# junyanz/interactive-deep-colorization

Hardware: NVIDIA H100
Metric: net_forward images/sec @256x256 (higher is better)
Workload: dtype f16x2-split operands, f32 accumulate (ab within 1e-3 of the f32 reference)

## Files before the change

include/idc_b200.h:

```cpp
#ifndef IDC_B200_H_
#define IDC_B200_H_

#include <stddef.h>
#include <stdint.h>

#ifdef __cplusplus
extern "C" {
#endif

typedef struct idc_ctx idc_ctx;

enum {
  IDC_OK = 0,
  IDC_ERR_ARG = -1,
  IDC_ERR_CUDA = -2,
  IDC_ERR_STATE = -3,
  IDC_ERR_KEY = -4,
  IDC_ERR_UNSUPPORTED = -5,
  IDC_ERR_WATCHDOG = -6,
  IDC_ERR_RANGE = -7
};

enum {
  IDC_FLAG_DIST = 1u << 0,
// ... 71 lines not shown
                         int mask_f32, int l_mode, const double* L, int h, int w, uint8_t* rgb, void* stream);

int idc_resize_u8_linear(int device, int h_src, int w_src, const uint8_t* src, int h_dst, int w_dst, uint8_t* dst,
                         void* stream);
int idc_cubic_lab2rgb_u8(int device, int h_in, int w_in, const double* ab, int h, int w, const double* L, uint8_t* rgb,
                         void* stream);
int idc_gamut_ab(int device, double L, int gamut_size, int D, uint8_t* rgb, uint8_t* mask, void* stream);

typedef struct { int64_t off; int32_t h, w; } idc_photo;
#define IDC_MAX_PHOTOS 128
#define IDC_MAX_PHOTO_SIDE 16777216
#define IDC_MAX_PHOTO_X 16384
int idc_photo_prep(int device, int n, const idc_photo* photos, const uint8_t* src, int X, float* L_mc, uint8_t* rgb,
                   void* stream);
int idc_photo_render(int device, int n, const idc_photo* photos, const uint8_t* src, int X, const double* lab,
                     uint8_t* out, void* stream);
int idc_hint_raster(int device, int n, int h, int w, int count, const void* block, float* ab, float* mask, void* stream);
int idc_rgb_sse(int device, int n, int h, int w, const uint8_t* a, const uint8_t* b, int64_t* sse, void* stream);

int idc_act_exponent(idc_ctx* ctx, const char* name, int* exp_out);
int idc_num_acts(idc_ctx* ctx);
const char* idc_act_name(idc_ctx* ctx, int i);
int idc_act_absmax(idc_ctx* ctx, const char* name, int n, float* out_host);
int idc_set_act_range(idc_ctx* ctx, const char* name, double max_abs);
int idc_get_activation(idc_ctx* ctx, const char* name, float* out_nchw, size_t out_floats,
                       int* c, int* h, int* w);
int idc_set_activation(idc_ctx* ctx, const char* name, int n, const float* in_nchw);
int idc_run_op(idc_ctx* ctx, const char* op_name, int n, void* stream);
int idc_num_ops(idc_ctx* ctx);
const char* idc_op_name(idc_ctx* ctx, int i);
int idc_set_profiling(idc_ctx* ctx, int enable);
int idc_get_profile(idc_ctx* ctx, float* ms, int max_slots);
double idc_op_flops(idc_ctx* ctx, int i);
int idc_last_launch_count(idc_ctx* ctx);
int idc_graph_captures(idc_ctx* ctx);
double idc_flops_per_image(idc_ctx* ctx);

const char* idc_last_error(idc_ctx* ctx);
int idc_destroy(idc_ctx* ctx);

#ifdef __cplusplus
}
#endif
#endif
```

interactive_deep_colorization_b200/_lib.py:

```python
import ctypes
import os

import numpy as np

_HERE = os.path.dirname(os.path.abspath(__file__))
LIB_PATH = os.path.join(_HERE, "lib", "libidc_b200.so")
if os.environ.get("IDC_B200_LIB"):
    LIB_PATH = os.environ["IDC_B200_LIB"]

IDC_OK = 0
ERR_ARG, ERR_CUDA, ERR_STATE, ERR_KEY, ERR_UNSUPPORTED, ERR_WATCHDOG, ERR_RANGE = -1, -2, -3, -4, -5, -6, -7
FLAG_DIST = 1 << 0
FLAG_ENGINE_SIMT = 1 << 1
FLAG_FAST_FP16 = 1 << 2
FLAG_GLOBAL_HINTS = 1 << 3
FLAG_NO_GRAPH = 1 << 4
FLAG_KEEP_CONV10 = 1 << 5
FLAG_CAFFE313 = 1 << 6
F32, F64, I64 = 0, 1, 2
MAX_HINTS = 1024
MAX_PHOTOS = 128
MAX_PHOTO_SIDE = 1 << 24
MAX_PHOTO_X = 16384
HINT_HDR_BYTES = 16
# ... 28 lines not shown
    ("idc_ab_reccs", _c.c_int, [_P, _c.c_int, _c.c_int, _c.c_int, _c.c_int, _c.c_int, _c.c_int, _P, _P, _P, _P]),
    ("idc_ab_reccs_pmf", _c.c_int, [_c.c_int, _P, _c.c_int, _c.c_int, _c.c_int, _P, _P, _P, _P]),
    ("idc_caffe313_pred_ab", _c.c_int, [_P, _c.c_int, _c.c_float, _P, _P]),
    ("idc_caffe313_dist_pixel", _c.c_int, [_P, _c.c_int, _c.c_int, _c.c_int, _c.c_float, _P]),
    ("idc_caffe313_dist_map", _c.c_int, [_P, _c.c_int, _c.c_float, _P, _P]),
    ("idc_negentropy", _c.c_int, [_c.c_int, _c.c_int, _c.c_int, _c.c_int, _P, _P, _P]),
    ("idc_dist_negentropy", _c.c_int, [_P, _c.c_int, _P]),
    ("idc_lab2rgb_u8", _c.c_int, [_c.c_int, _c.c_int, _c.c_int, _c.c_int, _P, _P, _P, _P]),
    ("idc_rgb2lab_f64", _c.c_int, [_c.c_int, _c.c_int, _c.c_int, _c.c_int, _P, _P, _P]),
    ("idc_global_stats", _c.c_int, [_c.c_int, _c.c_int, _c.c_int, _P, _P, _P, _P]),
    ("idc_zoom_lab2rgb_u8", _c.c_int, [_c.c_int, _c.c_int, _c.c_int, _P, _c.c_int, _c.c_int, _P, _P, _P]),
    ("idc_render_planes_u8", _c.c_int, [_c.c_int, _c.c_int, _c.c_int, _P, _c.c_int, _c.c_int, _P, _c.c_int, _c.c_int,
                                        _P, _c.c_int, _c.c_int, _P, _P]),
    ("idc_resize_u8_linear", _c.c_int, [_c.c_int, _c.c_int, _c.c_int, _P, _c.c_int, _c.c_int, _P, _P]),
    ("idc_cubic_lab2rgb_u8", _c.c_int, [_c.c_int, _c.c_int, _c.c_int, _P, _c.c_int, _c.c_int, _P, _P, _P]),
    ("idc_photo_prep", _c.c_int, [_c.c_int, _c.c_int, _P, _P, _c.c_int, _P, _P, _P]),
    ("idc_photo_render", _c.c_int, [_c.c_int, _c.c_int, _P, _P, _c.c_int, _P, _P, _P]),
    ("idc_hint_raster", _c.c_int, [_c.c_int, _c.c_int, _c.c_int, _c.c_int, _c.c_int, _P, _P, _P, _P]),
    ("idc_rgb_sse", _c.c_int, [_c.c_int, _c.c_int, _c.c_int, _c.c_int, _P, _P, _P, _P]),
    ("idc_get_activation", _c.c_int, [_P, _c.c_char_p, _P, _c.c_size_t, _c.POINTER(_c.c_int),
                                      _c.POINTER(_c.c_int), _c.POINTER(_c.c_int)]),
    ("idc_set_activation", _c.c_int, [_P, _c.c_char_p, _c.c_int, _P]),
    ("idc_act_exponent", _c.c_int, [_P, _c.c_char_p, _c.POINTER(_c.c_int)]),
    ("idc_num_acts", _c.c_int, [_P]),
    ("idc_act_name", _c.c_char_p, [_P, _c.c_int]),
    ("idc_act_absmax", _c.c_int, [_P, _c.c_char_p, _c.c_int, _c.POINTER(_c.c_float)]),
    ("idc_set_act_range", _c.c_int, [_P, _c.c_char_p, _c.c_double]),
    ("idc_run_op", _c.c_int, [_P, _c.c_char_p, _c.c_int, _P]),
    ("idc_num_ops", _c.c_int, [_P]),
    ("idc_op_name", _c.c_char_p, [_P, _c.c_int]),
    ("idc_set_profiling", _c.c_int, [_P, _c.c_int]),
    ("idc_get_profile", _c.c_int, [_P, _c.POINTER(_c.c_float), _c.c_int]),
    ("idc_op_flops", _c.c_double, [_P, _c.c_int]),
    ("idc_last_launch_count", _c.c_int, [_P]),
    ("idc_flops_per_image", _c.c_double, [_P]),
    ("idc_last_error", _c.c_char_p, [_P]),
    ("idc_destroy", _c.c_int, [_P]),
]

_lib = None


class IdcError(RuntimeError):
    def __init__(self, code, msg):
        RuntimeError.__init__(self, "idc_b200 error %d: %s" % (code, msg))
        self.code = code


def load():
    global _lib
    if _lib is not None:
        return _lib
    if not os.path.isfile(LIB_PATH):
        raise ImportError("libidc_b200.so not built (%s missing); run `python -c 'import __graft_entry__ as g; g.build()'` "
                          "or `make -C interactive_deep_colorization_b200/csrc`" % LIB_PATH)
    lib = ctypes.CDLL(LIB_PATH)
    for name, res, args in SYMBOLS:
        fn = getattr(lib, name)
        fn.restype = res
        fn.argtypes = args
    _lib = lib
    return lib


def check(ctx, rc):
    if rc != IDC_OK:
# ... 3 lines not shown
```

interactive_deep_colorization_b200/csrc/idc_api.cu:

```cuda
#include <math.h>
#include <stdarg.h>
#include <stdio.h>
#include <string.h>

#include <algorithm>
#include <cmath>

#include "idc_internal.h"

using namespace idc;

struct idc_ctx : public idc::Ctx {};

namespace {

int fail(Ctx* c, int code, const char* fmt, ...) {
  char buf[512];
  va_list ap;
  va_start(ap, fmt);
  vsnprintf(buf, sizeof(buf), fmt, ap);
  va_end(ap);
  if (c) c->err = buf;
  return code;
}
// ... 1572 lines not shown
  return IDC_OK;
}

int idc_get_profile(idc_ctx* c, float* ms, int max_slots) {
  if (!c || !ms) return IDC_ERR_ARG;
  const int slots = (int)c->ops.size() + 2;
  if (max_slots < slots) return fail(c, IDC_ERR_ARG, "need %d slots", slots);
  CUDA_TRY(c, cudaSetDevice(c->dev));
  CUDA_TRY(c, cudaDeviceSynchronize());
  const int rc = take_device_flags(c, "device pipeline watchdog fired (code %d)");
  if (rc != IDC_OK) return rc;
  for (int i = 0; i < slots; ++i) ms[i] = 0.f;
  int runs = 0;
  for (auto& ev : c->prof_runs) {
    if ((int)ev.size() == slots + 1) {
      for (int i = 0; i < slots; ++i) {
        float t = 0.f;
        cudaEventElapsedTime(&t, ev[i].get(), ev[i + 1].get());
        ms[i] += t;
      }
      runs++;
    }
    for (Event& e : ev) c->prof_pool.push_back(std::move(e));
  }
  c->prof_runs.clear();
  if (runs) for (int i = 0; i < slots; ++i) ms[i] /= runs;
  return slots;
}

double idc_op_flops(idc_ctx* c, int i) {
  return (c && i >= 0 && i < (int)c->ops.size()) ? c->ops[i].flops_per_image : 0.0;
}

extern "C" int idc_debug_graph_timing(idc_ctx* c, int enable, float* ms) {
  if (!c) return IDC_ERR_ARG;
  CUDA_TRY(c, cudaSetDevice(c->dev));
  if (enable && !c->dbg_ev[0].get()) {
    Event ev[2];
    CUDA_TRY(c, cudaEventCreate(ev[0].put()));
    CUDA_TRY(c, cudaEventCreate(ev[1].put()));
    c->dbg_ev[0] = std::move(ev[0]);
    c->dbg_ev[1] = std::move(ev[1]);
  }
  c->dbg_graph_timing = enable != 0 && c->dbg_ev[0].get();
  if (ms) *ms = c->dbg_graph_ms;
  return IDC_OK;
}

int idc_num_ops(idc_ctx* c) { return c ? (int)c->ops.size() : 0; }
const char* idc_op_name(idc_ctx* c, int i) {
  return (c && i >= 0 && i < (int)c->ops.size()) ? c->ops[i].name.c_str() : nullptr;
}
int idc_last_launch_count(idc_ctx* c) { return c ? c->launch_count : 0; }
int idc_graph_captures(idc_ctx* c) { return c ? c->graph_captures : 0; }

double idc_flops_per_image(idc_ctx* c) {
  if (!c) return 0;
  double f = 2.0 * c->H * c->W * 64.0 * 36.0 + 2.0 * c->H * c->W * 2.0 * 128.0;
  for (auto& op : c->ops) f += op.flops_per_image;
  return f;
}

const char* idc_last_error(idc_ctx* c) { return c ? c->err.c_str() : "null ctx"; }

int idc_destroy(idc_ctx* c) {
  if (!c) return IDC_ERR_ARG;
// ... 8 lines not shown
```

interactive_deep_colorization_b200/csrc/idc_internal.h:

```cpp
#pragma once
#include <cuda.h>
#include <cuda_fp16.h>
#include <cuda_runtime.h>
#include <stdint.h>

#include <map>
#include <memory>
#include <string>
#include <utility>
#include <vector>

#include "../../include/idc_b200.h"

namespace idc {

template <typename H, auto Release>
class Owner {
 public:
  Owner() = default;
  Owner(Owner&& o) noexcept { std::swap(h_, o.h_); }
  Owner& operator=(Owner&& o) noexcept { std::swap(h_, o.h_); return *this; }
  ~Owner() { reset(); }
  H get() const { return h_; }
  H* put() { reset(); return &h_; }
// ... 169 lines not shown
  Stream own_stream;
  std::unique_ptr<HostPipeStreams> pipe;
  std::unique_ptr<SideBranch> side;
  int image_n = 0;
  std::unique_ptr<HintBlock> hints;
  int graph_captures = 0;
  GraphExec graph_exec;
  const void* graph_ptrs[8] = {nullptr};
  float graph_maskcent = 0.f;
  int launch_count = 0;
  int graph_launches = 0;
  bool chain = false;
  bool gadd_active = false;
  int last_n = 0;
  DevMem<double> d_reccs;
  DevMem<float> d_negent;
  DevMem<float> d_dist313;
  bool dist_resident = false;
  int dist_valid_n = 0;
  bool click_mode = false;
  std::unique_ptr<ClickBlock> click;
  bool click_served = false;
  bool profiling = false;
  std::vector<std::vector<Event>> prof_runs;
  std::vector<Event> prof_pool;
  std::string err;
};

cudaError_t simt_run_op(Ctx* c, ConvOp& op, int n, cudaStream_t st);
int umma_plan_op(Ctx* c, ConvOp& op);
cudaError_t umma_run_op(Ctx* c, ConvOp& op, int n, float* out_ab_fused, float out_mult, cudaStream_t st, int img0 = 0,
                        int max_ctas = 0);
bool umma_op_uses_split_k(const ConvOp& op);

cudaError_t launch_conv1_1(Ctx* c, int n, const float* L, const float* ab, const float* mask,
                           float maskcent, cudaStream_t st, int img0 = 0);
cudaError_t launch_conv1_1_umma(Ctx* c, int n, const float* L, const float* ab, const float* mask, float maskcent,
                                cudaStream_t st, int img0 = 0);
cudaError_t conv1_1_umma_pack(Ctx* c);
constexpr size_t kHintHdrBytes = 16;
constexpr size_t kHintBlockBytes = kHintHdrBytes + (size_t)IDC_MAX_HINTS * sizeof(idc_hint);
cudaError_t launch_hint_raster(Ctx* c, int n, int H, int W, const char* hints_dev, float* ab, float* mask,
                               cudaStream_t st);
cudaError_t launch_gamut(double L, int gamut_size, int D, int A, uint8_t* rgb, uint8_t* mask, cudaStream_t st);
cudaError_t launch_out_head(Ctx* c, int n, float* out_ab, cudaStream_t st);
cudaError_t launch_softmax529(Ctx* c, int n, float* out_dist, cudaStream_t st);
cudaError_t launch_lab2rgb(Ctx* c, int n, int h, int w, const float* L, float l_offset, const float* ab,
                           uint8_t* rgb, cudaStream_t st, double* abq = nullptr);
cudaError_t launch_decode313(Ctx* c, int n, float T, float* out_ab, cudaStream_t st);
cudaError_t launch_dist313_pixel(Ctx* c, int img, int y, int x, float S, float* out313_dev, cudaStream_t st);
cudaError_t launch_dist313_map(Ctx* c, int n, float S, float* out_dev, cudaStream_t st);
cudaError_t launch_negentropy(int n, int bins, int hw, const float* dist, float* out, cudaStream_t st);
cudaError_t launch_ab_reccs(const float* pmf, size_t bin_stride, const float* pts_dev, int K, int max_iter,
                            int n_init, double* out_dev, cudaStream_t st, const int* dyn = nullptr);
cudaError_t launch_click_pmf(Ctx* c, const int* click_dev, int n_img, int* out_hdr, float* out_pmf, cudaStream_t st);
cudaError_t launch_global_stats(int h, int w, const uint8_t* rgb, const float* pts, float* out316, cudaStream_t st);
cudaError_t launch_rgb2lab(int n, int h, int w, const uint8_t* rgb, double* lab, cudaStream_t st);
cudaError_t launch_render_planes(const double* ab, int ab_order, int ab_f32, const double* mask, int mask_f32, int l_mode,
                                 const double* L, int hin, int win, int H, int W, uint8_t* rgb, cudaStream_t st);
cudaError_t launch_resize_linear_u8(const uint8_t* src, int hs, int ws, uint8_t* dst, int hd, int wd, cudaStream_t st);
cudaError_t launch_cubic_lab2rgb(const double* ab, int hin, int win, const double* L, int H, int W, uint8_t* rgb,
                                 cudaStream_t st);
cudaError_t launch_photo_prep(int n, const idc_photo* table, const uint8_t* src, int X, float* L_mc, uint8_t* rgb,
                              cudaStream_t st);
cudaError_t launch_photo_render(int n, const idc_photo* table, const uint8_t* src, int X, const double* lab, uint8_t* out,
                                cudaStream_t st);
// ... 155 lines not shown
```

interactive_deep_colorization_b200/csrc/idc_umma.cu:

```cuda
#include <stdio.h>
#include <stdlib.h>

#include "idc_internal.h"

namespace idc {

constexpr int kBM = 128;
constexpr int kBK = 64;
constexpr int kThreads = 384;
constexpr int kProdRegs = 40;
constexpr int kMathRegs = 232;
constexpr int kMathThreads = 256;

struct UmmaParams {
  const CUtensorMap* amaps;
  const int4* kblk;
  int nkb, ncls;
  int chunk_kb;
  int split_k;
  float* ws;
  int* counters;
  int n_img, tiles_y, tiles_x, n_tiles_n, total_tiles;
  int hbox, wbox, wshift;
  int Hl, Wl, cout_pad;
// ... 184 lines not shown
}
__device__ __forceinline__ bool f16_top(uint32_t m) {
  return ((m & 0xFFFFu) >= kF16MaxBits) | ((m >> 16) >= kF16MaxBits);
}

__device__ __forceinline__ void split_h(float v, __half& hi, __half& lo) {
  v = fminf(fmaxf(v, -65504.f), 65504.f);
  hi = __float2half_rn(v);
  lo = __float2half_rn(v - __half2float(hi));
}

__device__ __forceinline__ int frag_col(int i, int lane) { return 8 * (i >> 2) + 2 * (lane & 3) + (i & 1); }

constexpr int kHaloW = 10, kHaloH = 18;
constexpr int kHaloPlane = (kHaloW * kHaloH * 128 + 1023) / 1024 * 1024;


template <int BN, int MT, int CG, bool SPLIT, bool HALO>
struct SmemPlan {
  static constexpr int kABytes = MT * kBM * kBK * 2;
  static constexpr int kAStage = HALO ? 0 : kABytes;
  static constexpr int kBBytes = BN * kBK * 2;
  static constexpr int kStageBytes = (SPLIT ? 2 : 1) * (kAStage + kBBytes);
  static constexpr int kHaloSlot = (SPLIT ? 2 : 1) * kHaloPlane;
  static constexpr int kHaloBytes = HALO ? 2 * kHaloSlot : 0;
  static constexpr int kOutRow = 64 * 2 + 16;
  static constexpr int kOutWarp = 16 * kOutRow;
  static constexpr int kOutStage = 8 * kOutWarp;
  static constexpr int kTail = 3 * BN * 4 + 272 * 4 + 256;
  static constexpr int kBudget = 232448 - 1024 - kTail - kOutStage - kHaloBytes;
  static constexpr int kStages = kBudget / kStageBytes >= 4 ? 4 : kBudget / kStageBytes;
  static constexpr int kTotal = kStages * kStageBytes + kHaloBytes + kOutStage + kTail + 1024;
  static_assert(kStages >= 2, "need at least a double-buffered operand ring");
  static_assert(MT * BN <= 128, "register budget: chunk + tile accumulators of MT*BN columns per math thread pair");
  static_assert(!HALO || MT == 1, "halo tiles are single 16x8-pixel M-tiles");
  static_assert(CG == 1 || CG == 2, "clusters of one or two CTAs");
};

template <int BN, int MT, int CG, bool SPLIT, bool HALO>
__global__ void __launch_bounds__(kThreads, 1)
umma_conv_kernel(const __grid_constant__ CUtensorMap bmap_hi, const __grid_constant__ CUtensorMap bmap_lo,
                 const __grid_constant__ UmmaParams p) {
  using SP = SmemPlan<BN, MT, CG, SPLIT, HALO>;
  constexpr int STAGES = SP::kStages;
  constexpr int R = BN / 2;
  constexpr bool PAIR = CG == 2;
  extern __shared__ uint8_t smem_raw[];
  uint8_t* smem = reinterpret_cast<uint8_t*>((reinterpret_cast<uintptr_t>(smem_raw) + 1023) & ~uintptr_t(1023));
  uint8_t* s_halo = smem + STAGES * SP::kStageBytes;
  uint8_t* s_out = s_halo + SP::kHaloBytes;
  float* s_bias = reinterpret_cast<float*>(s_out + SP::kOutStage);
  float* s_scale = s_bias + BN;
  float* s_shift = s_scale + BN;
  float* s_head = s_shift + BN;
  uint64_t* full_bar = reinterpret_cast<uint64_t*>(s_head + 272);
  uint64_t* empty_bar = full_bar + 4;
  uint64_t* afull_bar = full_bar + 8;
  uint64_t* aempty_bar = full_bar + 10;

  const int warp = threadIdx.x >> 5, lane = threadIdx.x & 31;
  const uint32_t cta_rank = PAIR ? cluster_ctarank() : 0u;

  if (p.wout) {
    for (int i = threadIdx.x; i < 256; i += kThreads) s_head[i] = p.wout[i];
    if (threadIdx.x < 2) s_head[256 + threadIdx.x] = p.bout[threadIdx.x];
  }
  if (threadIdx.x == 32) {
    prefetch_tmap(&bmap_hi);
    if (SPLIT) prefetch_tmap(&bmap_lo);
    for (int i = 0; i < p.n_amaps; ++i) prefetch_tmap(p.amaps + i);
  }
  if (threadIdx.x == 0) {
    for (int s = 0; s < STAGES; ++s) {
      mbar_init(smem_u32(&full_bar[s]), 1);
      mbar_init(smem_u32(&empty_bar[s]), 8 * CG);
    }
    if (HALO)
      for (int a = 0; a < 2; ++a) {
        mbar_init(smem_u32(&afull_bar[a]), 1);
        mbar_init(smem_u32(&aempty_bar[a]), 8);
      }
    asm volatile("fence.mbarrier_init.release.cluster;" ::: "memory");
  }
  if (PAIR) cluster_sync_all(); else __syncthreads();
  pdl_launch_dependents();
  pdl_wait();

  const int tiles_per_img = p.tiles_y * p.tiles_x;
  const int S = p.split_k;
  const int n_items = p.total_tiles * S;
  const int w0 = blockIdx.x / CG, wstep = gridDim.x / CG;

  if (warp < 4) {
    asm volatile("setmaxnreg.dec.sync.aligned.u32 %0;" ::"n"(kProdRegs));
    if (warp == 0) {
      int stage = 0;
      uint32_t phase = 0;
      uint32_t hcount = 0;
      for (int w = w0; w < n_items; w += wstep) {
        const int tile = w / S, ks = w - tile * S;
        const int kbeg = (ks * p.nkb) / S, kend = ((ks + 1) * p.nkb) / S;
        int r = tile;
        const int nt = r % p.n_tiles_n;
        r /= p.n_tiles_n;
        const int cls = r % p.ncls;
        r /= p.ncls;
        if (PAIR) r = 2 * r + (int)cta_rank;
        const int img_rel = r / tiles_per_img;
        r -= img_rel * tiles_per_img;
        const int img = p.img0 + img_rel;
        const int y0 = (r / p.tiles_x) * (p.hbox * MT), x0 = (r % p.tiles_x) * p.wbox;
        const int brow = cls * p.cout_pad + nt * BN + (int)cta_rank * (BN / CG);
        const int4* kb = p.kblk + cls * p.nkb;
        for (int k = kbeg; k < kend; ++k) {
          if (HALO && k % 9 == 0) {
            const uint32_t slot = hcount & 1, hphase = (hcount >> 1) & 1;
            ++hcount;
            mbar_wait(smem_u32(&aempty_bar[slot]), hphase ^ 1, p.err, 6);
            if (elect_one()) {
              const uint32_t fa = smem_u32(&afull_bar[slot]);
              const uint32_t sh = smem_u32(s_halo + slot * SP::kHaloSlot);
              const int c0 = (k / 9) * kBK;
// ... 18 lines not shown
            }
            if (PAIR) {
              tma_load_2d_mc(sb, &bmap_hi, fb, kcol, brow);
              if (SPLIT) tma_load_2d_mc(sb + SP::kBBytes, &bmap_lo, fb, kcol, brow);
            } else {
              tma_load_2d(sb, &bmap_hi, fb, kcol, brow);
              if (SPLIT) tma_load_2d(sb + SP::kBBytes, &bmap_lo, fb, kcol, brow);
            }
          }
          __syncwarp();
          if (++stage == STAGES) { stage = 0; phase ^= 1; }
        }
      }
    }
  } else {
    asm volatile("setmaxnreg.inc.sync.aligned.u32 %0;" ::"n"(kMathRegs));
    const int et = threadIdx.x - 128;
    const int wg = et >> 7;
    const int wi = (et >> 5) & 3;
    const uint32_t wbuf = smem_u32(s_out) + (uint32_t)(et >> 5) * SP::kOutWarp;
    auto release = [&](uint64_t* bar) {
      __syncwarp();
      if (lane == 0) {
        mbar_arrive(smem_u32(bar));
        if (PAIR) mbar_arrive_remote(smem_u32(bar), cta_rank ^ 1u);
      }
    };
    int stage = 0;
    uint32_t phase = 0;
    uint32_t hcount = 0;
    int staged_key = -1;
    bool sat = false;
    for (int w = w0; w < n_items; w += wstep) {
      const int tile = w / S, ks = w - tile * S;
      const int kbeg = (ks * p.nkb) / S, kend = ((ks + 1) * p.nkb) / S;
      int r = tile;
      const int nt = r % p.n_tiles_n;
      r /= p.n_tiles_n;
      const int cls = r % p.ncls;
      r /= p.ncls;
      if (PAIR) r = 2 * r + (int)cta_rank;
      const int img_rel = r / tiles_per_img;
      r -= img_rel * tiles_per_img;
      const int img = p.img0 + img_rel;
      const int ty0 = (r / p.tiles_x) * (p.hbox * MT), tx0 = (r % p.tiles_x) * p.wbox;
      const int n0 = nt * BN;
      const int vkey = p.gadd ? (img * p.n_tiles_n + nt) : nt;
      if (vkey != staged_key) {
        asm volatile("bar.sync 1, 256;" ::: "memory");
        for (int i = et; i < BN; i += kMathThreads) {
          s_bias[i] = p.bias[n0 + i];
          s_scale[i] = p.scale[n0 + i];
          const int gi = img < p.n_img ? img : p.n_img - 1;
          s_shift[i] = p.shift[n0 + i] + (p.gadd ? p.gadd[(size_t)gi * p.gadd_ld + n0 + i] * p.gadd_mult : 0.f);
        }
        asm volatile("bar.sync 1, 256;" ::: "memory");
        staged_key = vkey;
      }

      float acc[MT][R];
#pragma unroll
      for (int m = 0; m < MT; ++m)
#pragma unroll
        for (int j = 0; j < R; ++j) acc[m][j] = 0.f;
      for (int k0 = kbeg; k0 < kend; k0 += p.chunk_kb) {
        const int k1 = (k0 + p.chunk_kb < kend) ? k0 + p.chunk_kb : kend;
        float part[MT][R];
#pragma unroll
        for (int m = 0; m < MT; ++m)
#pragma unroll
          for (int j = 0; j < R; ++j) part[m][j] = 0.f;
        int prev = -1;
        for (int k = k0; k < k1; ++k) {
          uint32_t hslot = 0;
          if (HALO) {
            if (k % 9 == 0) {
              mbar_wait(smem_u32(&afull_bar[hcount & 1]), (hcount >> 1) & 1, p.err, 7);
              ++hcount;
            }
            hslot = (hcount - 1) & 1;
          }
          mbar_wait(smem_u32(&full_bar[stage]), phase, p.err, 3);
          const uint32_t st0 = smem_u32(smem + stage * SP::kStageBytes);
          const uint32_t sb = st0 + (SPLIT ? 2 : 1) * SP::kAStage;
          const uint64_t b_hi = make_sw128_desc(sb), b_lo = make_sw128_desc(sb + SP::kBBytes);
          uint32_t ha = 0;
          if (HALO) {
            const int4 e = __ldg(p.kblk + k);
            ha = smem_u32(s_halo + hslot * SP::kHaloSlot) + (uint32_t)((e.z + wg * 8) * kHaloW + e.w) * 128u;
          }
          wgmma_fence();
#pragma unroll
          for (int m = 0; m < MT; ++m) {
            const uint32_t sa = st0 + (uint32_t)(wg * MT + m) * (64 * 128);
            const uint64_t a_hi = HALO ? make_sw128_desc(ha, kHaloW * 128) : make_sw128_desc(sa);
            const uint64_t a_lo = HALO ? make_sw128_desc(ha + kHaloPlane, kHaloW * 128) : make_sw128_desc(sa + SP::kABytes);
            uint32_t first = (k == k0) ? 0u : 1u;
// ... 58 lines not shown
          if (q == ks) continue;
          const float* rp = p.ws + (size_t)(tile * S + q) * R * kMathThreads + et;
#pragma unroll
          for (int i = 0; i < R; ++i)
            if ((i >> 4) % S == ks) acc[0][i] += __ldcg(rp + (size_t)i * kMathThreads);
        }
      }

      const float neg_slope = p.act == ACT_RELU ? 0.f : (p.act == ACT_LEAKY02 ? 0.2f : 1.f);
      unsigned own = ~0u;
      if (S > 1) {
        own = 0u;
#pragma unroll
        for (int pc = 0; pc < BN / 32; ++pc) own |= (pc % S == ks ? 1u : 0u) << pc;
      }
#pragma unroll
      for (int m = 0; m < MT; ++m) {
        const int blk = (wg * MT + m) * 64;
#pragma unroll
        for (int i = 0; i < R; ++i) {
          const int c = frag_col(i, lane);
          const float t = acc[m][i] + s_bias[c];
          acc[m][i] = fmaf(fmaxf(t, neg_slope * t), s_scale[c], s_shift[c]);
        }
        int ry[2], rx[2];
        bool ok[2];
#pragma unroll
        for (int h = 0; h < 2; ++h) {
          const int rr = blk + wi * 16 + (lane >> 2) + 8 * h;
          ry[h] = ty0 + (rr >> p.wshift);
          rx[h] = tx0 + (rr & (p.wbox - 1));
          ok[h] = ry[h] < p.Hl && rx[h] < p.Wl && img < p.n_img;
        }
        if (p.wout) {
          float h0[2] = {0.f, 0.f}, h1[2] = {0.f, 0.f};
#pragma unroll
          for (int i = 0; i < R; ++i) {
            const int c = frag_col(i, lane), h = (i >> 1) & 1;
            h0[h] = fmaf(acc[m][i], s_head[c], h0[h]);
            h1[h] = fmaf(acc[m][i], s_head[128 + c], h1[h]);
          }
#pragma unroll
          for (int h = 0; h < 2; ++h) {
#pragma unroll
            for (int o = 1; o <= 2; o <<= 1) {
              h0[h] += __shfl_xor_sync(0xffffffffu, h0[h], o);
              h1[h] += __shfl_xor_sync(0xffffffffu, h1[h], o);
            }
            if ((lane & 3) == 0 && ok[h]) {
              const size_t HW = (size_t)p.Hl * p.Wl;
              const size_t o = (size_t)img * 2 * HW + (size_t)ry[h] * p.Wl + rx[h];
              p.out_ab[o] = tanhf(h0[h] + s_head[256]) * p.out_mult;
              p.out_ab[o + HW] = tanhf(h1[h] + s_head[257]) * p.out_mult;
            }
          }
        } else if (p.out_f32) {
#pragma unroll
          for (int i = 0; i < R; i += 2) {
            const int h = (i >> 1) & 1;
            if ((S > 1 && (i >> 4) % S != ks) || !ok[h]) continue;
            float* o = p.out_f32 + ((size_t)(img * p.Hl + ry[h]) * p.Wl + rx[h]) * p.out_ld + n0 + frag_col(i, lane);
            *reinterpret_cast<float2*>(o) = make_float2(acc[m][i], acc[m][i + 1]);
          }
        } else {
          __half* prow[4];
          const int rl0 = lane >> 3, ch = lane & 7;
#pragma unroll
// ... 350 lines not shown
  PFN_encodeTiled enc = get_encode();
  if (!enc) { c->err = "cuTensorMapEncodeTiled entry point not available"; return IDC_ERR_CUDA; }
  op.umma_plan.reset();
  std::unique_ptr<UmmaPlan, UmmaPlanFree> pl(new UmmaPlan());
  pl->num_sms = c->num_sms;
  pl->dev = c->dev;
  op.bn_tile = (op.cout_pad % 128 == 0) ? 128 : 64;
  if (op.cout_pad % op.bn_tile) { c->err = "cout not tileable: " + op.name; return IDC_ERR_ARG; }
  if (op.fuse_out_head && op.cout_pad != 128) { c->err = "fused model_out needs 128 columns: " + op.name; return IDC_ERR_ARG; }
  int best = 1 << 30;
  for (int wb = 128; wb >= 8; wb >>= 1) {
    const int hb = kBM / wb;
    const int t = ceil_div(op.Wl, wb) * ceil_div(op.Hl, hb);
    if (t < best) { best = t; op.wbox = wb; op.hbox = hb; }
  }
  {
    const int mode = c->opt.halo;
    bool ok = mode >= 1 && !c->fast && op.ncls == 1 && op.ntaps == 9;
    unsigned seen = 0;
    for (int t = 0; ok && t < op.ntaps; ++t) {
      const Tap& tp = op.taps[0][t];
      if (tp.src != op.taps[0][0].src || op.src[tp.src].s != 1 || tp.ty < -1 || tp.ty > 1 || tp.tx < -1 || tp.tx > 1) ok = false;
      else seen |= 1u << ((tp.ty + 1) * 3 + tp.tx + 1);
    }
    if (ok && (seen != 0x1FFu || op.src[op.taps[0][0].src].cin % kBK)) ok = false;
    if (ok && !(op.bn_tile == 128 || (mode >= 3 && op.bn_tile == 64))) ok = false;
    if (ok) {
      const long T = (long)c->max_n * ceil_div(op.Hl, 16) * ceil_div(op.Wl, 8) * (op.cout_pad / op.bn_tile);
      if (T < 2L * pl->num_sms && mode < 3) ok = false;
    }
    pl->halo = ok;
    if (ok) { op.wbox = 8; op.hbox = 16; }
  }
  pl->mt = 1;
  if (op.bn_tile == 64 && !pl->halo && !op.fuse_out_head) {
    const long tiles2 = (long)op.ncls * c->max_n * ceil_div(op.Hl, 2 * op.hbox) * ceil_div(op.Wl, op.wbox) *
                        (op.cout_pad / op.bn_tile);
    if (tiles2 >= 2L * pl->num_sms) pl->mt = 2;
  }
  {
    const int v = c->opt.mt;
    if (!pl->halo && v == 1) pl->mt = 1;
    if (!pl->halo && v == 2 && !op.fuse_out_head) { pl->mt = 2; op.bn_tile = 64; }
  }
  pl->cg = 1;
  {
    const long tiles_mt = (long)op.ncls * c->max_n * ceil_div(op.Hl, op.hbox * pl->mt) * ceil_div(op.Wl, op.wbox) *
                          (op.cout_pad / op.bn_tile);
    const int mode = c->opt.pairs;
    if (!c->fast && (mode >= 2 || (mode == 1 && tiles_mt >= 2L * pl->num_sms))) pl->cg = 2;
  }
  const int nkb = op.K / kBK;
  {
    const int ty = ceil_div(op.Hl, op.hbox * pl->mt), tx = ceil_div(op.Wl, op.wbox), ntn = op.cout_pad / op.bn_tile;
    const long T = (long)op.ncls * c->max_n * ty * tx * ntn;
    const bool eligible = nkb >= 8 && !op.fuse_out_head && pl->mt == 1 && pl->cg == 1 && !pl->halo;
    int S = 1;
    if (T * 2 <= pl->num_sms && eligible) {
      S = (int)(pl->num_sms / T);
      if (S > nkb / 4) S = nkb / 4;
      if (S > op.bn_tile / 32) S = op.bn_tile / 32;
      if (S < 1) S = 1;
    }
    {
      const int v = c->opt.split_k;
      if (eligible && v >= 1 && v <= nkb && v <= op.bn_tile / 32 && T * v <= pl->num_sms) S = v;
    }
    pl->split_k = S;
    pl->ws_tiles = (int)T;
    pl->ws_floats = S > 1 ? (size_t)T * S * kBM * op.bn_tile : 0;
    if (pl->ws_floats > c->splitk_ws_floats) c->splitk_ws_floats = pl->ws_floats;
    if (S > 1 && pl->ws_tiles > c->splitk_max_tiles) c->splitk_max_tiles = pl->ws_tiles;
  }
  std::vector<ViewKey> views;
  std::vector<int4> kblk((size_t)op.ncls * nkb);
  if (pl->halo) {
    const int src = op.taps[0][0].src, groups = op.src[src].cin / kBK;
    views.push_back(ViewKey{src, 1, 0, 0});
    for (int i = 0; i < nkb; ++i) {
      const int g = i / 9, t = i % 9;
      kblk[i] = make_int4(0, (t * groups + g) * kBK, op.taps[0][t].ty + 1, op.taps[0][t].tx + 1);
    }
  }
// ... 40 lines not shown
        char msg[256];
        snprintf(msg, sizeof(msg), "cuTensorMapEncodeTiled(A) failed (%d) for op %s view %zu", (int)r, op.name.c_str(), i);
        c->err = msg;
        return IDC_ERR_CUDA;
      }
    }
  }
  for (int part = 0; part < 2; ++part) {
    cuuint64_t dims[2] = {(cuuint64_t)op.K, (cuuint64_t)op.ncls * op.cout_pad};
    cuuint64_t strides[1] = {(cuuint64_t)op.K * 2};
    cuuint32_t box[2] = {(cuuint32_t)kBK, (cuuint32_t)(op.bn_tile / pl->cg)};
    cuuint32_t estr[2] = {1, 1};
    CUresult r = enc(part == 0 ? &pl->bmap_hi : &pl->bmap_lo, CU_TENSOR_MAP_DATA_TYPE_FLOAT16, 2,
                     part == 0 ? (void*)op.w_hi : (void*)op.w_lo, dims, strides, box, estr,
                     CU_TENSOR_MAP_INTERLEAVE_NONE, CU_TENSOR_MAP_SWIZZLE_128B, CU_TENSOR_MAP_L2_PROMOTION_L2_256B,
                     CU_TENSOR_MAP_FLOAT_OOB_FILL_NONE);
    if (r != CUDA_SUCCESS) {
      char msg[256];
      snprintf(msg, sizeof(msg), "cuTensorMapEncodeTiled(B) failed (%d) for op %s", (int)r, op.name.c_str());
      c->err = msg;
      return IDC_ERR_CUDA;
    }
  }
  if (cudaMalloc(pl->d_amaps.put(), amaps.size() * sizeof(CUtensorMap)) != cudaSuccess ||
      cudaMalloc(pl->d_kblk.put(), kblk.size() * sizeof(int4)) != cudaSuccess ||
      cudaMemcpy(pl->d_amaps.get(), amaps.data(), amaps.size() * sizeof(CUtensorMap), cudaMemcpyHostToDevice) != cudaSuccess ||
      cudaMemcpy(pl->d_kblk.get(), kblk.data(), kblk.size() * sizeof(int4), cudaMemcpyHostToDevice) != cudaSuccess) {
    c->err = "uploading the launch plan failed in umma_plan_op: " + op.name;
    return IDC_ERR_CUDA;
  }

  UmmaParams& q = pl->prm;
  q.amaps = pl->d_amaps.get(); q.n_amaps = (int)amaps.size(); q.kblk = pl->d_kblk.get(); q.nkb = nkb; q.ncls = op.ncls;
  {
    const int natural = (op.cout_pad % 256 == 0) ? 256 : (op.cout_pad % 192 == 0) ? 192 : (op.cout_pad % 128 == 0) ? 128 : 64;
    int g = c->fast ? 4 : (natural <= 128 ? 2 : 1);
    if (c->opt.chunk_kb >= 1) g = c->opt.chunk_kb;
    q.chunk_kb = g;
  }
  q.tiles_y = ceil_div(op.Hl, op.hbox * pl->mt); q.tiles_x = ceil_div(op.Wl, op.wbox);
  q.n_tiles_n = op.cout_pad / op.bn_tile;
  q.hbox = op.hbox; q.wbox = op.wbox;
  q.wshift = 0;
  while ((1 << q.wshift) < op.wbox) q.wshift++;
  q.Hl = op.Hl; q.Wl = op.Wl; q.cout_pad = op.cout_pad;
  q.bias = op.epi.bias; q.scale = op.epi.scale; q.shift = op.epi.shift;
  q.gadd = nullptr; q.gadd_ld = 512; q.gadd_mult = op.out_buf >= 0 ? ldexpf(1.f, c->bufs[op.out_buf].exp) : 1.f;
  q.act = op.epi.act;
  if (op.out_f32) {
    q.out_f32 = op.out_f32_ptr; q.out_ld = op.cout_pad;
  } else if (op.out_buf >= 0) {
    const ActBuf& ob = c->bufs[op.out_buf];
    q.out_hi = (__half*)ob.p0.get(); q.out_lo = (__half*)ob.p1.get();
    q.Hout = ob.H; q.Wout = ob.W; q.Cout = ob.C; q.os = op.os;
  }
  if (op.fuse_out_head) { q.wout = c->wout; q.bout = c->bout; }
  q.err = c->d_err;
  q.range = c->d_range; q.range_bit = op.out_buf >= 0 ? 1u << op.out_buf : 0u;
  q.img0 = 0;
  op.umma_plan = std::move(pl);
  return IDC_OK;
}

void UmmaPlanFree::operator()(UmmaPlan* p) const { delete p; }

bool umma_op_uses_split_k(const ConvOp& op) {
  return op.umma_plan && op.umma_plan->split_k > 1;
}

cudaError_t umma_run_op(Ctx* c, ConvOp& op, int n, float* out_ab_fused, float out_mult, cudaStream_t st, int img0,
                        int max_ctas) {
  const UmmaPlan* pl = op.umma_plan.get();
  if (!pl) return cudaErrorInvalidValue;
  UmmaParams prm = pl->prm;
  prm.max_ctas = (max_ctas > 0 && pl->split_k == 1) ? (max_ctas / pl->cg) * pl->cg : 0;
  prm.img0 = img0;
  prm.n_img = img0 + n;
  if (img0 && pl->split_k > 1) return cudaErrorInvalidValue;
  const int m_tiles = n * prm.tiles_y * prm.tiles_x;
  prm.total_tiles = op.ncls * (pl->cg == 2 ? (m_tiles + 1) / 2 : m_tiles) * prm.n_tiles_n;
  prm.gadd = (op.epi.gadd && c->gadd_active) ? c->gvec.get() : nullptr;
  prm.out_ab = out_ab_fused;
  prm.split_k = pl->split_k;
  prm.ws = c->splitk_ws.get();
  prm.counters = c->splitk_counters.get();
  if (pl->split_k > 1 && (!prm.ws || !prm.counters)) return cudaErrorInvalidValue;
  prm.out_mult = out_mult;
  if (op.fuse_out_head && !out_ab_fused) return cudaErrorInvalidValue;
  c->launch_count++;
  const bool pdl = pdl_take(c);
  const bool split = !c->fast;
  if (pl->halo) {
    if (!split) return cudaErrorInvalidValue;
    switch (op.bn_tile * 10 + pl->cg) {
      case 641: return launch_inst<64, 1, 1, true, true>(*pl, prm, st, pdl);
      case 642: return launch_inst<64, 1, 2, true, true>(*pl, prm, st, pdl);
      case 1281: return launch_inst<128, 1, 1, true, true>(*pl, prm, st, pdl);
      case 1282: return launch_inst<128, 1, 2, true, true>(*pl, prm, st, pdl);
      default: return cudaErrorInvalidValue;
    }
  }
#define IDC_LAUNCH(BN_, MT_, CG_) \
  return split ? launch_inst<BN_, MT_, CG_, true>(*pl, prm, st, pdl) : launch_inst<BN_, MT_, CG_, false>(*pl, prm, st, pdl)
  switch (op.bn_tile * 100 + pl->mt * 10 + pl->cg) {
    case 6411: IDC_LAUNCH(64, 1, 1);
    case 6421: IDC_LAUNCH(64, 2, 1);
    case 12811: IDC_LAUNCH(128, 1, 1);
    case 6412: return launch_inst<64, 1, 2, true>(*pl, prm, st, pdl);
    case 6422: return launch_inst<64, 2, 2, true>(*pl, prm, st, pdl);
    case 12812: return launch_inst<128, 1, 2, true>(*pl, prm, st, pdl);
    default: break;
  }
#undef IDC_LAUNCH
  return cudaErrorInvalidValue;
}

}
```

interactive_deep_colorization_b200/engine.py:

```python
import ctypes
import json
import math
import os

import numpy as np

from . import _lib


def _np_ptr(a):
    return ctypes.c_void_p(a.ctypes.data)


def as_hints(rects):
    if isinstance(rects, np.ndarray) and rects.dtype.names:
        out = np.empty(rects.shape[0], _lib.HINT_DTYPE)
        for f in _lib.HINT_DTYPE.names:
            out[f] = rects[f]
        return out
    return np.array([tuple(r) for r in rects], dtype=_lib.HINT_DTYPE).reshape(-1)


ACT_BUFFERS = ("a1_1", "conv1_2", "a2_1", "conv2_2", "a3_1", "a3_2", "conv3_3", "a4_1", "a4_2", "conv4_3",
               "a5_1", "a5_2", "conv5_3", "a6_1", "a6_2", "conv6_3", "a7_1", "a7_2", "conv7_3",
# ... 379 lines not shown
    def act_absmax(self, name, n):
        v = ctypes.c_float()
        _lib.check(self.h, self.lib.idc_act_absmax(self.h, name.encode(), int(n), ctypes.byref(v)))
        return v.value

    def get_activation(self, name, n):
        import torch
        c, h, w = self.activation_shape(name)
        out = torch.empty((n, c, h, w), dtype=torch.float32, device="cuda:%d" % self.device)
        _lib.check(self.h, self.lib.idc_get_activation(self.h, name.encode(), out.data_ptr(), out.numel(), None, None, None))
        return out

    def set_activation(self, name, t):
        assert t.is_cuda and t.is_contiguous()
        _lib.check(self.h, self.lib.idc_set_activation(self.h, name.encode(), t.shape[0], t.data_ptr()))

    def run_op(self, op_name, n):
        import torch
        st = torch.cuda.current_stream(self.device).cuda_stream
        _lib.check(self.h, self.lib.idc_run_op(self.h, op_name.encode(), n, st))

    def set_profiling(self, on):
        _lib.check(self.h, self.lib.idc_set_profiling(self.h, 1 if on else 0))

    def get_profile(self):
        names = ["pack+conv1_1"] + self.op_names() + ["heads+post"]
        buf = (ctypes.c_float * len(names))()
        rc = self.lib.idc_get_profile(self.h, buf, len(names))
        if rc < 0:
            _lib.check(self.h, rc)
        flops = [2.0 * self.H * self.W * 64 * 36] + [self.lib.idc_op_flops(self.h, i) for i in range(len(names) - 2)] + [0.0]
        return [(names[i], float(buf[i]), flops[i]) for i in range(len(names))]

    def last_launch_count(self):
        return self.lib.idc_last_launch_count(self.h)

    def flops_per_image(self):
        return self.lib.idc_flops_per_image(self.h)

    def close(self):
        if getattr(self, "h", None):
            self.lib.idc_destroy(self.h)
            self.h = None
            for p in getattr(self, "_pinned", []):
                self.lib.idc_host_free(p)
            self._pinned = []

    def __del__(self):
        try:
            self.close()
        except Exception:
            pass
```

Baseline: 1397.

## Add tall MT=2 BN=128 conv tiles with per-M-tile chunk loop

```diff
diff --git a/include/idc_b200.h b/include/idc_b200.h
--- a/include/idc_b200.h
+++ b/include/idc_b200.h
@@ -127,6 +127,8 @@
 int idc_set_profiling(idc_ctx* ctx, int enable);
 int idc_get_profile(idc_ctx* ctx, float* ms, int max_slots);
 double idc_op_flops(idc_ctx* ctx, int i);
+#define IDC_PLAN_FIELDS 11
+int idc_op_plan(idc_ctx* ctx, int i, int* out, int n);
 int idc_last_launch_count(idc_ctx* ctx);
 int idc_graph_captures(idc_ctx* ctx);
 double idc_flops_per_image(idc_ctx* ctx);
diff --git a/interactive_deep_colorization_b200/_lib.py b/interactive_deep_colorization_b200/_lib.py
--- a/interactive_deep_colorization_b200/_lib.py
+++ b/interactive_deep_colorization_b200/_lib.py
@@ -84,6 +84,7 @@
     ("idc_set_profiling", _c.c_int, [_P, _c.c_int]),
     ("idc_get_profile", _c.c_int, [_P, _c.POINTER(_c.c_float), _c.c_int]),
     ("idc_op_flops", _c.c_double, [_P, _c.c_int]),
+    ("idc_op_plan", _c.c_int, [_P, _c.c_int, _c.POINTER(_c.c_int), _c.c_int]),
     ("idc_last_launch_count", _c.c_int, [_P]),
     ("idc_flops_per_image", _c.c_double, [_P]),
     ("idc_last_error", _c.c_char_p, [_P]),
diff --git a/interactive_deep_colorization_b200/csrc/idc_api.cu b/interactive_deep_colorization_b200/csrc/idc_api.cu
--- a/interactive_deep_colorization_b200/csrc/idc_api.cu
+++ b/interactive_deep_colorization_b200/csrc/idc_api.cu
@@ -1628,6 +1628,14 @@
   return (c && i >= 0 && i < (int)c->ops.size()) ? c->ops[i].flops_per_image : 0.0;
 }
 
+int idc_op_plan(idc_ctx* c, int i, int* out, int n) {
+  if (!c || i < 0 || i >= (int)c->ops.size() || !out) return IDC_ERR_ARG;
+  if (c->simt) return fail(c, IDC_ERR_UNSUPPORTED, "the SIMT engine has no wgmma plan");
+  if (!c->weights_ready) return fail(c, IDC_ERR_STATE, "weights not finalized");
+  const int rc = umma_op_plan(c->ops[i], !c->fast, out, n);
+  return rc < 0 ? fail(c, rc, "idc_op_plan needs %d ints", kPlanFields) : rc;
+}
+
 extern "C" int idc_debug_graph_timing(idc_ctx* c, int enable, float* ms) {
   if (!c) return IDC_ERR_ARG;
   CUDA_TRY(c, cudaSetDevice(c->dev));
diff --git a/interactive_deep_colorization_b200/csrc/idc_internal.h b/interactive_deep_colorization_b200/csrc/idc_internal.h
--- a/interactive_deep_colorization_b200/csrc/idc_internal.h
+++ b/interactive_deep_colorization_b200/csrc/idc_internal.h
@@ -225,6 +225,8 @@
 cudaError_t umma_run_op(Ctx* c, ConvOp& op, int n, float* out_ab_fused, float out_mult, cudaStream_t st, int img0 = 0,
                         int max_ctas = 0);
 bool umma_op_uses_split_k(const ConvOp& op);
+constexpr int kPlanFields = IDC_PLAN_FIELDS;
+int umma_op_plan(const ConvOp& op, bool split, int* out, int n);
 
 cudaError_t launch_conv1_1(Ctx* c, int n, const float* L, const float* ab, const float* mask,
                            float maskcent, cudaStream_t st, int img0 = 0);
diff --git a/interactive_deep_colorization_b200/csrc/idc_umma.cu b/interactive_deep_colorization_b200/csrc/idc_umma.cu
--- a/interactive_deep_colorization_b200/csrc/idc_umma.cu
+++ b/interactive_deep_colorization_b200/csrc/idc_umma.cu
@@ -240,7 +240,9 @@
   static constexpr int kStages = kBudget / kStageBytes >= 4 ? 4 : kBudget / kStageBytes;
   static constexpr int kTotal = kStages * kStageBytes + kHaloBytes + kOutStage + kTail + 1024;
   static_assert(kStages >= 2, "need at least a double-buffered operand ring");
-  static_assert(MT * BN <= 128, "register budget: chunk + tile accumulators of MT*BN columns per math thread pair");
+  static constexpr bool kTall = MT == 2 && BN == 128;
+  static_assert(MT * BN / 2 + (kTall ? BN / 2 : MT * BN / 2) <= 192,
+                "register budget: tile + chunk accumulators per math thread, out of 232");
   static_assert(!HALO || MT == 1, "halo tiles are single 16x8-pixel M-tiles");
   static_assert(CG == 1 || CG == 2, "clusters of one or two CTAs");
 };
@@ -295,7 +297,7 @@
   pdl_wait();
 
   const int tiles_per_img = p.tiles_y * p.tiles_x;
-  const int S = p.split_k;
+  const int S = (MT == 1 && CG == 1 && !HALO) ? p.split_k : 1;
   const int n_items = p.total_tiles * S;
   const int w0 = blockIdx.x / CG, wstep = gridDim.x / CG;
 
@@ -380,19 +382,23 @@
     int staged_key = -1;
     bool sat = false;
     for (int w = w0; w < n_items; w += wstep) {
-      const int tile = w / S, ks = w - tile * S;
-      const int kbeg = (ks * p.nkb) / S, kend = ((ks + 1) * p.nkb) / S;
-      int r = tile;
-      const int nt = r % p.n_tiles_n;
-      r /= p.n_tiles_n;
-      const int cls = r % p.ncls;
-      r /= p.ncls;
-      if (PAIR) r = 2 * r + (int)cta_rank;
-      const int img_rel = r / tiles_per_img;
-      r -= img_rel * tiles_per_img;
-      const int img = p.img0 + img_rel;
-      const int ty0 = (r / p.tiles_x) * (p.hbox * MT), tx0 = (r % p.tiles_x) * p.wbox;
-      const int n0 = nt * BN;
+      int tile, ks, kbeg, kend, nt, cls, img, ty0, tx0, n0;
+      auto locate = [&](int wi_) {
+        tile = wi_ / S; ks = wi_ - tile * S;
+        kbeg = (ks * p.nkb) / S; kend = ((ks + 1) * p.nkb) / S;
+        int r = tile;
+        nt = r % p.n_tiles_n;
+        r /= p.n_tiles_n;
+        cls = r % p.ncls;
+        r /= p.ncls;
+        if (PAIR) r = 2 * r + (int)cta_rank;
+        const int img_rel = r / tiles_per_img;
+        r -= img_rel * tiles_per_img;
+        img = p.img0 + img_rel;
+        ty0 = (r / p.tiles_x) * (p.hbox * MT); tx0 = (r % p.tiles_x) * p.wbox;
+        n0 = nt * BN;
+      };
+      locate(w);
       const int vkey = p.gadd ? (img * p.n_tiles_n + nt) : nt;
       if (vkey != staged_key) {
         asm volatile("bar.sync 1, 256;" ::: "memory");
@@ -411,6 +417,60 @@
       for (int m = 0; m < MT; ++m)
 #pragma unroll
         for (int j = 0; j < R; ++j) acc[m][j] = 0.f;
+      if constexpr (SP::kTall) {
+        float part[R];
+#pragma unroll
+        for (int j = 0; j < R; ++j) part[j] = 0.f;
+        for (int k0 = kbeg; k0 < kend; k0 += p.chunk_kb) {
+          const int nk = (k0 + p.chunk_kb < kend ? k0 + p.chunk_kb : kend) - k0;
+#pragma unroll
+          for (int m = 0; m < MT; ++m) {
+#pragma unroll 1
+            for (int j = 0; j < nk; ++j) {
+              const int s = stage + j < STAGES ? stage + j : stage + j - STAGES;
+              if (m == 0) mbar_wait(smem_u32(&full_bar[s]), stage + j < STAGES ? phase : phase ^ 1u, p.err, 3);
+              const uint32_t st0 = smem_u32(smem + s * SP::kStageBytes);
+              const uint32_t sb = st0 + (SPLIT ? 2 : 1) * SP::kAStage;
+              const uint64_t b_hi = make_sw128_desc(sb), b_lo = make_sw128_desc(sb + SP::kBBytes);
+              const uint32_t sa = st0 + (uint32_t)(wg * MT + m) * (64 * 128);
+              const uint64_t a_hi = make_sw128_desc(sa), a_lo = make_sw128_desc(sa + SP::kABytes);
+              uint32_t first = j == 0 ? 0u : 1u;
+              wgmma_fence();
+              if (SPLIT) {
+#pragma unroll
+                for (int kk = 0; kk < kBK / 16; ++kk) {
+                  const uint64_t adv = (uint64_t)(kk * 2);
+                  wgmma_n128(part, a_lo + adv, b_hi + adv, first);
+                  wgmma_n128(part, a_hi + adv, b_lo + adv, 1u);
+                  first = 1u;
+                }
+              }
+#pragma unroll
+              for (int kk = 0; kk < kBK / 16; ++kk) {
+                const uint64_t adv = (uint64_t)(kk * 2);
+                wgmma_n128(part, a_hi + adv, b_hi + adv, first);
+                first = 1u;
+              }
+              wgmma_commit();
+              if (m == MT - 1 && j > 0) {
+                wgmma_wait<1>();
+                release(&empty_bar[s == 0 ? STAGES - 1 : s - 1]);
+              }
+            }
+            wgmma_wait<0>();
+            wgmma_reg_fence(part);
+#pragma unroll
+            for (int j = 0; j < R; ++j) acc[m][j] += part[j];
+          }
+          const int last = stage + nk - 1;
+          release(&empty_bar[last < STAGES ? last : last - STAGES]);
+          stage += nk;
+          if (stage >= STAGES) { stage -= STAGES; phase ^= 1u; }
+        }
+        int w_again = w;
+        asm volatile("" : "+r"(w_again));
+        locate(w_again);
+      } else
       for (int k0 = kbeg; k0 < kend; k0 += p.chunk_kb) {
         const int k1 = (k0 + p.chunk_kb < kend) ? k0 + p.chunk_kb : kend;
         float part[MT][R];
@@ -535,7 +595,7 @@
           rx[h] = tx0 + (rr & (p.wbox - 1));
           ok[h] = ry[h] < p.Hl && rx[h] < p.Wl && img < p.n_img;
         }
-        if (p.wout) {
+        if (MT == 1 && p.wout) {
           float h0[2] = {0.f, 0.f}, h1[2] = {0.f, 0.f};
 #pragma unroll
           for (int i = 0; i < R; ++i) {
@@ -952,8 +1012,15 @@
     pl->halo = ok;
     if (ok) { op.wbox = 8; op.hbox = 16; }
   }
+  int chunk_kb;
+  {
+    const int natural = (op.cout_pad % 256 == 0) ? 256 : (op.cout_pad % 192 == 0) ? 192 : (op.cout_pad % 128 == 0) ? 128 : 64;
+    chunk_kb = c->fast ? 4 : (natural <= 128 ? 2 : 1);
+    if (c->opt.chunk_kb >= 1) chunk_kb = c->opt.chunk_kb;
+  }
+  const int tall_stages = c->fast ? SmemPlan<128, 2, 1, false, false>::kStages : SmemPlan<128, 2, 1, true, false>::kStages;
   pl->mt = 1;
-  if (op.bn_tile == 64 && !pl->halo && !op.fuse_out_head) {
+  if (!pl->halo && !op.fuse_out_head && op.bn_tile == 128 && chunk_kb == 1) {
     const long tiles2 = (long)op.ncls * c->max_n * ceil_div(op.Hl, 2 * op.hbox) * ceil_div(op.Wl, op.wbox) *
                         (op.cout_pad / op.bn_tile);
     if (tiles2 >= 2L * pl->num_sms) pl->mt = 2;
@@ -961,7 +1028,10 @@
   {
     const int v = c->opt.mt;
     if (!pl->halo && v == 1) pl->mt = 1;
-    if (!pl->halo && v == 2 && !op.fuse_out_head) { pl->mt = 2; op.bn_tile = 64; }
+    if (!pl->halo && v == 2 && !op.fuse_out_head) {
+      pl->mt = 2;
+      if (chunk_kb > tall_stages) op.bn_tile = 64;
+    }
   }
   pl->cg = 1;
   {
@@ -969,6 +1039,10 @@
                           (op.cout_pad / op.bn_tile);
     const int mode = c->opt.pairs;
     if (!c->fast && (mode >= 2 || (mode == 1 && tiles_mt >= 2L * pl->num_sms))) pl->cg = 2;
+    if (pl->cg == 2 && pl->mt == 2 && op.bn_tile == 128) {
+      if (c->opt.mt == 2) op.bn_tile = 64;
+      else pl->mt = 1;
+    }
   }
   const int nkb = op.K / kBK;
   {
@@ -1075,12 +1149,7 @@
 
   UmmaParams& q = pl->prm;
   q.amaps = pl->d_amaps.get(); q.n_amaps = (int)amaps.size(); q.kblk = pl->d_kblk.get(); q.nkb = nkb; q.ncls = op.ncls;
-  {
-    const int natural = (op.cout_pad % 256 == 0) ? 256 : (op.cout_pad % 192 == 0) ? 192 : (op.cout_pad % 128 == 0) ? 128 : 64;
-    int g = c->fast ? 4 : (natural <= 128 ? 2 : 1);
-    if (c->opt.chunk_kb >= 1) g = c->opt.chunk_kb;
-    q.chunk_kb = g;
-  }
+  q.chunk_kb = chunk_kb;
   q.tiles_y = ceil_div(op.Hl, op.hbox * pl->mt); q.tiles_x = ceil_div(op.Wl, op.wbox);
   q.n_tiles_n = op.cout_pad / op.bn_tile;
   q.hbox = op.hbox; q.wbox = op.wbox;
@@ -1111,6 +1180,34 @@
   return op.umma_plan && op.umma_plan->split_k > 1;
 }
 
+template <int BN, int MT, bool SPLIT, bool HALO>
+static void stage_info(int* stages, int* bytes) {
+  using SP = SmemPlan<BN, MT, 1, SPLIT, HALO>;
+  *stages = SP::kStages;
+  *bytes = SP::kStageBytes;
+}
+
+int umma_op_plan(const ConvOp& op, bool split, int* out, int n) {
+  const UmmaPlan* pl = op.umma_plan.get();
+  if (!pl || !out || n < kPlanFields) return IDC_ERR_ARG;
+  using F = void (*)(int*, int*);
+  static const F tab[2][2][2] = {
+      {{stage_info<64, 1, false, false>, stage_info<64, 1, true, false>},
+       {stage_info<64, 2, false, false>, stage_info<64, 2, true, false>}},
+      {{stage_info<128, 1, false, false>, stage_info<128, 1, true, false>},
+       {stage_info<128, 2, false, false>, stage_info<128, 2, true, false>}}};
+  int stages = 0, stage_bytes = 0;
+  if (pl->halo) (op.bn_tile == 128 ? stage_info<128, 1, true, true> : stage_info<64, 1, true, true>)(&stages, &stage_bytes);
+  else tab[op.bn_tile == 128][pl->mt == 2][split](&stages, &stage_bytes);
+  const UmmaParams& q = pl->prm;
+  const long long halo_bytes = pl->halo ? (long long)(q.nkb / 9) * (split ? 2 : 1) * kHaloW * kHaloH * 128 : 0;
+  const int v[kPlanFields] = {op.bn_tile, pl->mt, pl->cg, pl->split_k, pl->halo ? 1 : 0, stages, stage_bytes,
+                              q.chunk_kb, q.nkb, q.ncls * q.tiles_y * q.tiles_x * q.n_tiles_n,
+                              (int)(((long long)q.nkb * stage_bytes + halo_bytes) >> 10)};
+  for (int i = 0; i < kPlanFields; ++i) out[i] = v[i];
+  return kPlanFields;
+}
+
 cudaError_t umma_run_op(Ctx* c, ConvOp& op, int n, float* out_ab_fused, float out_mult, cudaStream_t st, int img0,
                         int max_ctas) {
   const UmmaPlan* pl = op.umma_plan.get();
@@ -1120,6 +1217,7 @@
   prm.img0 = img0;
   prm.n_img = img0 + n;
   if (img0 && pl->split_k > 1) return cudaErrorInvalidValue;
+  if (pl->split_k > 1 && (pl->mt != 1 || pl->cg != 1 || pl->halo)) return cudaErrorInvalidValue;
   const int m_tiles = n * prm.tiles_y * prm.tiles_x;
   prm.total_tiles = op.ncls * (pl->cg == 2 ? (m_tiles + 1) / 2 : m_tiles) * prm.n_tiles_n;
   prm.gadd = (op.epi.gadd && c->gadd_active) ? c->gvec.get() : nullptr;
@@ -1149,6 +1247,7 @@
     case 6411: IDC_LAUNCH(64, 1, 1);
     case 6421: IDC_LAUNCH(64, 2, 1);
     case 12811: IDC_LAUNCH(128, 1, 1);
+    case 12821: IDC_LAUNCH(128, 2, 1);
     case 6412: return launch_inst<64, 1, 2, true>(*pl, prm, st, pdl);
     case 6422: return launch_inst<64, 2, 2, true>(*pl, prm, st, pdl);
     case 12812: return launch_inst<128, 1, 2, true>(*pl, prm, st, pdl);
diff --git a/interactive_deep_colorization_b200/engine.py b/interactive_deep_colorization_b200/engine.py
--- a/interactive_deep_colorization_b200/engine.py
+++ b/interactive_deep_colorization_b200/engine.py
@@ -435,6 +435,17 @@
         flops = [2.0 * self.H * self.W * 64 * 36] + [self.lib.idc_op_flops(self.h, i) for i in range(len(names) - 2)] + [0.0]
         return [(names[i], float(buf[i]), flops[i]) for i in range(len(names))]
 
+    PLAN_FIELDS = ("bn", "mt", "cg", "split_k", "halo", "stages", "stage_bytes", "chunk_kb", "nkb", "tiles_per_image",
+                   "operand_kib_per_tile")
+
+    def op_plan(self, op_name):
+        i = self.op_names().index(op_name)
+        out = (ctypes.c_int * len(self.PLAN_FIELDS))()
+        rc = self.lib.idc_op_plan(self.h, i, out, len(out))
+        if rc < 0:
+            _lib.check(self.h, rc)
+        return dict(zip(self.PLAN_FIELDS, out))
+
     def last_launch_count(self):
         return self.lib.idc_last_launch_count(self.h)
 
```

After: 1422, median of 6. +1.7%, better.
